# KyanChen/RSPrompter

Hardware: NVIDIA H100
Metric: images/sec (higher is better)
Workload: dtype bf16

## Files before the change

### include/rsp_b200.h

```cpp
#ifndef RSP_B200_H_
#define RSP_B200_H_

#include <stdint.h>

#ifdef __cplusplus
extern "C" {
#endif

#define RSP_ABI_VERSION 2

int rsp_abi_version(void);
const char* rsp_last_error(void);

int rsp_gemm_bf16(const void* A, int lda, const void* W, int ldw, void* out, int ldo, int M, int N,
                  int K, const float* bias, const void* residual, int ldr, int res_fp32, int res_mod,
                  const int32_t* row_map, int act, int out_fp32, void* stream);

int rsp_conv3x3_nhwc_bf16(const void* x, int B, int H, int W, int C, const void* Wt, int ldw, void* out, int ldo,
                          int N, const float* bias, const void* residual, int ldr, int res_fp32, int act,
                          int out_fp32, void* stream);
int rsp_conv3x3_geometry_ok(int B, int H, int W, int C);

int rsp_gemm_bf16_simt(const void* A, int lda, const void* W, int ldw, void* out, int ldo, int M,
                       int N, int K, const float* bias, const void* residual, int ldr, int res_fp32,
// ... 33 lines not shown
                      void* stream);

int rsp_token_self_attention(const void* q, const void* k, const void* v, void* out, int N, int T,
                             int heads, int c, void* stream);
int rsp_t2i_attention(const void* q, const void* K, const void* V, int ldkv, const int32_t* kv_block, void* out,
                      int N, int Tq, int HW, void* stream);
int rsp_i2t_attention(const void* Q, const int32_t* q_block, const void* ktok, const void* vtok,
                      void* out, int N, int Tq, int HW, void* stream);

int rsp_t2i_fused(const void* keys, int ldk, const void* kvw, const float* kvb, const void* pe_kv, const void* q,
                  void* out, int N, int Tq, int HW, void* stream);

int rsp_i2t_fused(const void* keys, int ldk, const void* wq, const float* qb, const void* pe_q, const void* ktok,
                  const void* vtok, const void* wo, const float* ob, const float* ln_g, const float* ln_b, float eps,
                  void* out, int N, int Tq, int HW, void* stream);


int rsp_rpn_decode(const float* head_out, int ld, const int64_t* topk_idx, int K, int B, int H, int W,
                   int A, int stride, const float* base_anchors, const float* stds4, float img_h, float img_w,
                   float min_size, int out_off, int out_ld, float* boxes, float* scores, void* stream);
int rsp_rpn_decode_shapes(const float* head_out, int ld, const int64_t* topk_idx, int K, int B, int H, int W, int A,
                          int stride, const float* base_anchors, const float* stds4, const float* img_shapes,
                          float min_size, int out_off, int out_ld, float* boxes, float* scores, void* stream);

int rsp_bbox_cls_decode(const float* cls, int ld_cls, const float* reg, int ld_reg, const float* rois,
                        const uint8_t* roi_valid, int n, int C, const float* stds4, float img_h, float img_w,
                        float score_thr, float* scores, float* boxes, int64_t* labels, void* stream);
int rsp_bbox_cls_decode_shapes(const float* cls, int ld_cls, const float* reg, int ld_reg, const float* rois,
                               const uint8_t* roi_valid, int n, int C, const float* stds4, const float* img_shapes,
                               float score_thr, float* scores, float* boxes, int64_t* labels, void* stream);
// ... 115 lines not shown
```

### profiles/decoder_bench.py

```python
#!/usr/bin/env python
from __future__ import annotations

import argparse
import collections
import json
import os
import subprocess
import sys

ROOT = os.path.dirname(os.path.dirname(os.path.abspath(__file__)))
if ROOT not in sys.path:
    sys.path.insert(0, ROOT)

import torch

from rsprompter_b200 import _lib, synthetic
from rsprompter_b200.sam_config import SamDecoderArch
from rsprompter_b200.sam_decoder import SamMaskDecoderB200

NQ = 100


def _card() -> dict:
    q = subprocess.run(["nvidia-smi", "--query-gpu=name,power.limit,clocks.max.sm", "--format=csv,noheader"],
# ... 57 lines not shown
    N, Tq, C = ktok.shape
    return 4.0 * N * Tq * hw * C, Q.shape[0] * C * 2 + N * hw * C * 2


def _t2i_fused_cost(q, keys, kvw, kvb, pe_kv, hw):
    N, Tq, C = q.shape
    return 2.0 * keys.shape[0] * 256 * 256 + 4.0 * N * Tq * hw * C, keys.shape[0] * 256 * 2 + 2 * _nb(q)


def _i2t_fused_cost(keys, wq, qb, pe_q, ktok, vtok, wo, ob, ln, hw):
    N, Tq, C = ktok.shape
    R = keys.shape[0]
    return 2.0 * R * 256 * 128 * 2 + 4.0 * N * Tq * hw * C, R * 256 * 2 * 2


def _family(name: str, args, kw, n_img_rows: int) -> str:
    if name == "gemm":
        a, w = args[0], args[1]
        if a.shape[0] < n_img_rows:
            return "token-side gemm"
        if kw.get("ln64_gelu") is not None:
            return "up1 gemm (LN64 + GELU)"
        if kw.get("ln") is not None:
            return "i2t out_proj gemm (+ LN4)"
        if w.shape[0] == 256:
            return "t2i k|v gemm"
        return "i2t q gemm"
    return {"gemm_upscale_mask": "up2 gemm (GELU + hyper)", "t2i_attention": "t2i attention",
            "i2t_attention": "i2t attention", "t2i_fused": "t2i fused (k|v gemm + attention)",
            "i2t_fused": "i2t fused (q gemm + attention + out_proj + LN4)"}.get(name, "token-side " + name)


COSTS = {"gemm": _gemm_cost, "gemm_upscale_mask": _upscale_cost, "t2i_attention": _t2i_cost,
         "i2t_attention": _i2t_cost, "t2i_fused": _t2i_fused_cost, "i2t_fused": _i2t_fused_cost}
WRAPPED = ("gemm", "gemm_upscale_mask", "t2i_attention", "i2t_attention", "t2i_fused", "i2t_fused", "add_cast_bf16",
           "cast_bf16", "token_self_attention")


def per_family(run, n_img_rows: int, iters: int) -> dict:
    calls = []
    orig = {k: getattr(_lib, k) for k in WRAPPED if hasattr(_lib, k)}

    def wrap(name, fn):
        def inner(*args, **kw):
            s, e = torch.cuda.Event(enable_timing=True), torch.cuda.Event(enable_timing=True)
            s.record()
            out = fn(*args, **kw)
            e.record()
            cost = COSTS[name](*args, **kw) if name in COSTS else (0.0, 0)
            calls.append((_family(name, args, kw, n_img_rows), s, e, cost))
            return out
# ... 82 lines not shown
```

### rsprompter_b200/_lib.py

```python
from __future__ import annotations

import ctypes
import os
import subprocess
from pathlib import Path

import torch

_PKG_DIR = Path(__file__).resolve().parent
LIB_PATH = _PKG_DIR / "librsp_b200.so"
CSRC_DIR = _PKG_DIR / "csrc"


class RspError(RuntimeError):
    """Raised when an ``rsp_*`` entry point returns a non-zero status."""


def build_library(verbose: bool = False) -> Path:
    cmd = ["make", "-C", str(CSRC_DIR), "-j", str(os.cpu_count() or 4), "all"]
    res = subprocess.run(cmd, capture_output=True, text=True)
    if res.returncode != 0:
        raise RuntimeError(f"building librsp_b200.so failed:\n{res.stdout[-4000:]}\n{res.stderr[-4000:]}")
    if verbose:
        print(res.stdout[-2000:])
# ... 23 lines not shown
    "rsp_layernorm": ([_vp, _i, _i, _vp, _i, _i, _vp, _vp, _vp, _i, _i, _f, _i, _vp, _i, _vp], _i),
    "rsp_patchify16": ([_vp, _vp, _i, _i, _i, _vp], _i),
    "rsp_layernorm_add": ([_vp, _vp, _i, _vp, _i, _vp, _vp, _vp, _vp, _i, _vp, ctypes.c_longlong, _i, _f, _vp], _i),
    "rsp_im2col_nhwc": ([_vp, _vp, _i, _i, _i, _i, _i, _i, _i, _i, _vp], _i),
    "rsp_nhwc_to_nchw": ([_vp, _i, _vp, _i, _i, _i, _vp], _i),
    "rsp_cast_f32_bf16": ([_vp, _vp, ctypes.c_longlong, _vp], _i),
    "rsp_add_table_bf16": ([_vp, _vp, _vp, ctypes.c_longlong, ctypes.c_longlong, _vp], _i),
    "rsp_gemm_bf16_ex": ([_vp, _i, _vp, _i, _vp, _i, _i, _i, _i, _vp, _vp, _i, _i, _i, _vp, _i, _i,
                          _i, _vp, _vp, _f, _vp, _i, _vp, _vp, _i, _i, _vp], _i),
    "rsp_add_cast_bf16": ([_vp, _vp, _vp, ctypes.c_longlong, ctypes.c_longlong, _vp], _i),
    "rsp_token_self_attention": ([_vp, _vp, _vp, _vp, _i, _i, _i, _i, _vp], _i),
    "rsp_t2i_attention": ([_vp, _vp, _vp, _i, _vp, _vp, _i, _i, _i, _vp], _i),
    "rsp_i2t_attention": ([_vp, _vp, _vp, _vp, _vp, _i, _i, _i, _vp], _i),
    "rsp_t2i_fused": ([_vp, _i, _vp, _vp, _vp, _vp, _vp, _i, _i, _i, _vp], _i),
    "rsp_i2t_fused": ([_vp, _i, _vp, _vp, _vp, _vp, _vp, _vp, _vp, _vp, _vp, _f, _vp, _i, _i, _i, _vp], _i),
    "rsp_rpn_decode": ([_vp, _i, _vp, _i, _i, _i, _i, _i, _i, _vp, _vp, _f, _f, _f, _i, _i, _vp, _vp, _vp], _i),
    "rsp_bbox_cls_decode": ([_vp, _i, _vp, _i, _vp, _vp, _i, _i, _vp, _f, _f, _f, _vp, _vp, _vp, _vp], _i),
    "rsp_rpn_decode_shapes": ([_vp, _i, _vp, _i, _i, _i, _i, _i, _i, _vp, _vp, _vp, _f, _i, _i, _vp, _vp, _vp], _i),
    "rsp_nms_batched_topk": ([_vp, _vp, _vp, _i, _i, _f, _vp, _vp, _vp, _i, _vp], _i),
    "rsp_bbox_cls_decode_shapes": ([_vp, _i, _vp, _i, _vp, _vp, _i, _i, _vp, _vp, _f, _vp, _vp, _vp, _vp], _i),
    "rsp_nms_batched": ([_vp, _vp, _vp, _i, _i, _f, _vp, _vp, _vp, _vp], _i),
    "rsp_compact_keep": ([_vp, _vp, _vp, _vp, _i, _i, _i, _vp, _vp, _vp, _vp, _vp, _vp], _i),
    "rsp_roi_align_nhwc": ([_vp, _vp, _vp, _vp, _vp, _i, _vp, _i, _i, _i, _f, _vp, _vp], _i),
    "rsp_mask_paste": ([_vp, _vp, _i, _i, _i, _i, _i, _f, _i, _vp], _i),
    "rsp_pool2_nhwc": ([_vp, _vp, _i, _i, _i, _i, _i, _vp], _i),
    "rsp_zero_border_nhwc": ([_vp, _i, _i, _i, _i, _vp], _i),
    "rsp_sigmoid_f32": ([_vp, _vp, ctypes.c_longlong, _vp], _i),
    "rsp_mask_paste_boxes": ([_vp, _vp, _vp, _i, _i, _i, _i, _i, _f, _i, _vp], _i),
    "rsp_groupnorm_nhwc": ([_vp, _vp, _vp, _vp, _vp, _vp, _i, _i, _i, _i, _i, _f, _i, _vp], _i),
    "rsp_ms_deform_attn_sample": ([_vp, _vp, _i, _vp, _vp, _i, _i, _i, _i, _vp, _vp], _i),
# ... 272 lines not shown
    assert C == 128 and hw % 64 == 0
    assert keys.dtype == torch.bfloat16 and keys.dim() == 2 and keys.stride(1) == 1 and keys.shape == (N * hw, 256)
    for t, shape in ((wq, (128, 256)), (pe_q, (hw, 128)), (ktok, (N, Tq, 128)), (vtok, (N, Tq, 128)), (wo, (256, 128))):
        assert t.dtype == torch.bfloat16 and t.shape == shape and t.is_contiguous()
    for t, n in ((qb, 128), (ob, 256), (g, 256), (b, 256)):
        assert t.dtype == torch.float32 and t.numel() == n and t.is_contiguous()
    out = torch.empty((N * hw, 256), device=keys.device, dtype=torch.bfloat16)
    _check(_lib.rsp_i2t_fused(_ptr(keys), keys.stride(0), _ptr(wq), _ptr(qb), _ptr(pe_q), _ptr(ktok), _ptr(vtok),
                              _ptr(wo), _ptr(ob), _ptr(g), _ptr(b), float(eps), _ptr(out), N, Tq, hw, _stream()),
           "rsp_i2t_fused")
    launch_count += 1
    _log("gemm", 2.0 * N * hw * 256 * 256)
    return out


def i2t_attention(Q: torch.Tensor, ktok: torch.Tensor, vtok: torch.Tensor, hw: int,
                  q_block: torch.Tensor | None = None) -> torch.Tensor:
    global launch_count
    _require_cuda(Q, ktok, vtok, q_block)
    N, Tq, C = ktok.shape
    assert C == 128 and Q.dtype == torch.bfloat16 and Q.is_contiguous() and Q.shape[1] == 128
    assert ktok.dtype == torch.bfloat16 and vtok.dtype == torch.bfloat16
    assert ktok.is_contiguous() and vtok.is_contiguous() and vtok.shape == ktok.shape
    if q_block is not None:
        assert q_block.dtype == torch.int32 and q_block.numel() == N and q_block.is_contiguous()
    else:
        assert Q.shape[0] == N * hw
    out = torch.empty((N * hw, 128), device=Q.device, dtype=torch.bfloat16)
    _check(_lib.rsp_i2t_attention(_ptr(Q), _ptr(q_block), _ptr(ktok), _ptr(vtok), _ptr(out), N, Tq, hw, _stream()),
           "rsp_i2t_attention")
# ... 811 lines not shown
```

### rsprompter_b200/csrc/abi.cu

```cuda
#include "../../include/rsp_b200.h"

#include "attention.h"
#include "gemm.h"
#include "rowops.h"

namespace rsp { const char* last_error(); }
using namespace rsp;

static inline cudaStream_t S(void* s) { return static_cast<cudaStream_t>(s); }

extern "C" {

int rsp_abi_version(void) { return RSP_ABI_VERSION; }
const char* rsp_last_error(void) { return rsp::last_error(); }

static GemmArgs make_gemm_args(const void* A, int lda, const void* W, int ldw, void* out, int ldo,
                               int M, int N, int K, const float* bias, const void* residual, int ldr,
                               int res_fp32, int res_mod, const int32_t* row_map, int act,
                               int out_fp32) {
  GemmArgs a;
  a.A = A; a.lda = lda; a.W = W; a.ldw = ldw; a.out = out; a.ldo = ldo;
  a.M = M; a.N = N; a.K = K; a.bias = bias; a.residual = residual; a.ldr = ldr;
  a.res_fp32 = res_fp32; a.res_mod = res_mod; a.row_map = row_map; a.act = act;
  a.out_fp32 = out_fp32;
// ... 146 lines not shown
                      void* out, int N, int Tq, int HW, void* stream) {
  return i2t_attention(Q, q_block, ktok, vtok, out, N, Tq, HW, S(stream));
}

int rsp_t2i_fused(const void* keys, int ldk, const void* kvw, const float* kvb, const void* pe_kv, const void* q,
                  void* out, int N, int Tq, int HW, void* stream) {
  return t2i_fused(keys, ldk, kvw, kvb, pe_kv, q, out, N, Tq, HW, S(stream));
}

int rsp_i2t_fused(const void* keys, int ldk, const void* wq, const float* qb, const void* pe_q, const void* ktok,
                  const void* vtok, const void* wo, const float* ob, const float* ln_g, const float* ln_b, float eps,
                  void* out, int N, int Tq, int HW, void* stream) {
  return i2t_fused(keys, ldk, wq, qb, pe_q, ktok, vtok, wo, ob, ln_g, ln_b, eps, out, N, Tq, HW, S(stream));
}

}

#include "detect.h"

extern "C" {

int rsp_rpn_decode(const float* head_out, int ld, const int64_t* topk_idx, int K, int B, int H, int W,
                   int A, int stride, const float* base_anchors, const float* stds4, float img_h, float img_w,
                   float min_size, int out_off, int out_ld, float* boxes, float* scores, void* stream) {
  return rpn_decode(head_out, ld, reinterpret_cast<const long long*>(topk_idx), K, B, H, W, A, stride,
                    base_anchors, stds4, img_h, img_w, nullptr, min_size, out_off, out_ld, boxes, scores, S(stream));
}

int rsp_rpn_decode_shapes(const float* head_out, int ld, const int64_t* topk_idx, int K, int B, int H, int W, int A,
                          int stride, const float* base_anchors, const float* stds4, const float* img_shapes,
// ... 222 lines not shown
```

### rsprompter_b200/csrc/decoder.cu

```cuda
#include "decoder.h"
#include "sm90.cuh"

namespace rsp {

__device__ __forceinline__ void unpack8(const uint4& u, float (&f)[8]) {
  const uint32_t w[4] = {u.x, u.y, u.z, u.w};
#pragma unroll
  for (int j = 0; j < 4; ++j) {
    const __nv_bfloat162 h = *reinterpret_cast<const __nv_bfloat162*>(&w[j]);
    f[2 * j] = __bfloat162float(h.x);
    f[2 * j + 1] = __bfloat162float(h.y);
  }
}

__global__ void add_cast_bf16_kernel(const float* __restrict__ a, const float* __restrict__ b,
                                     __nv_bfloat16* __restrict__ out, long long n, long long b_mod) {
  const long long i = (static_cast<long long>(blockIdx.x) * blockDim.x + threadIdx.x) * 4;
  if (i >= n) return;
  float4 x = *reinterpret_cast<const float4*>(a + i);
  if (b) {
    const float4 y = *reinterpret_cast<const float4*>(b + (b_mod > 0 ? i % b_mod : i));
    x.x += y.x; x.y += y.y; x.z += y.z; x.w += y.w;
  }
  *reinterpret_cast<uint2*>(out + i) = make_uint2(pack_bf16x2(x.x, x.y), pack_bf16x2(x.z, x.w));
// ... 769 lines not shown
  static bool attr_set_dev[kMaxDevices] = {};
  bool& attr_set = attr_set_dev[current_device()];
  if (!attr_set) {
    RSP_CHECK_CUDA(cudaFuncSetAttribute(i2t_fused_kernel, cudaFuncAttributeMaxDynamicSharedMemorySize, IF_SMEM));
    attr_set = true;
  }
  const int num_tiles = static_cast<int>(M / IF_TILE);
  const int grid = num_tiles < num_sms() ? num_tiles : num_sms();
  i2t_fused_kernel<<<grid, IF_THREADS, IF_SMEM, stream>>>(
      tk, to, tq, tw, qb, static_cast<const __nv_bfloat16*>(pe_q), static_cast<const __nv_bfloat16*>(ktok),
      static_cast<const __nv_bfloat16*>(vtok), ob, ln_g, ln_b, eps, Tq, HW, num_tiles, 0.25f);
  RSP_CHECK_LAUNCH();
  return RSP_OK;
}

}
```

### rsprompter_b200/csrc/decoder.h

```cpp
#pragma once
#include "host_util.h"

namespace rsp {

int add_cast_bf16(const float* a, const float* b, void* out, long long n, long long b_mod,
                  cudaStream_t stream);
int token_self_attention(const void* q, const void* k, const void* v, void* out, int N, int T,
                         int heads, int c, cudaStream_t stream);
int t2i_attention(const void* q, const void* K, const void* V, int ldkv, const int* kv_block, void* out, int N,
                  int Tq, int HW, cudaStream_t stream);
int t2i_fused(const void* keys, int ldk, const void* kvw, const float* kvb, const void* pe_kv, const void* q,
              void* out, int N, int Tq, int HW, cudaStream_t stream);
int i2t_attention(const void* Q, const int* q_block, const void* ktok, const void* vtok, void* out,
                  int N, int Tq, int HW, cudaStream_t stream);
int i2t_fused(const void* keys, int ldk, const void* wq, const float* qb, const void* pe_q, const void* ktok,
              const void* vtok, const void* wo, const float* ob, const float* ln_g, const float* ln_b, float eps,
              void* out, int N, int Tq, int HW, cudaStream_t stream);

}
```

### rsprompter_b200/csrc/gemm_v2.cu

```cuda
#include <cstdlib>

#include "gemm.h"
#include "sm90.cuh"

namespace rsp {

namespace v2 {

constexpr int BM = 128;
constexpr int BK = 64;
constexpr int A_BYTES = BM * BK * 2;
constexpr int STG_ROW = 136;
constexpr int STG_WARP = 32 * STG_ROW;
constexpr int BAR_BYTES = 256;
constexpr int SMEM_MAX = 227 * 1024;

enum { EPI_STD = 0, EPI_LN_ROW = 1, EPI_LN64_GELU = 2, EPI_GELU_HYPER = 3 };

template <int BN, int EPI>
struct Cfg {
  static constexpr bool SPLIT = EPI == EPI_STD;
  static_assert(!SPLIT || BN <= 128, "a 64 x 256 wgmma needs more registers than a 512-thread block has per thread");
  static constexpr int THREADS = SPLIT ? 512 : 384;
  static constexpr int EPI_WARPS = SPLIT ? 4 : 8;
// ... 80 lines not shown
    float hyp[32];
    {
      const float4* h4 = reinterpret_cast<const float4*>(p.hyper + static_cast<size_t>(n) * 32);
#pragma unroll
      for (int i = 0; i < 8; ++i) {
        const float4 h = __ldg(h4 + i);
        hyp[4 * i] = h.x; hyp[4 * i + 1] = h.y; hyp[4 * i + 2] = h.z; hyp[4 * i + 3] = h.w;
      }
    }
    const uint32_t t_row = acc_row(acc_base, C::ACC_LD, q * 32 + lane) + 4 * hf * 64;
    float m2[2];
#pragma unroll
    for (int t = 0; t < 2; ++t) {
      uint32_t r[32];
      acc_ld32(t_row + (t * 32) * 4, r);
      const float4* b4 = reinterpret_cast<const float4*>(p.bias + hf * 64 + t * 32);
      float acc = 0.f;
#pragma unroll
      for (int i = 0; i < 8; ++i) {
        const float4 b = __ldg(b4 + i);
        acc += gelu_fast(__uint_as_float(r[4 * i]) + b.x) * hyp[4 * i];
        acc += gelu_fast(__uint_as_float(r[4 * i + 1]) + b.y) * hyp[4 * i + 1];
        acc += gelu_fast(__uint_as_float(r[4 * i + 2]) + b.z) * hyp[4 * i + 2];
        acc += gelu_fast(__uint_as_float(r[4 * i + 3]) + b.w) * hyp[4 * i + 3];
      }
      m2[t] = acc;
    }
    if (valid) {
      const int W4 = 4 * p.grid_w;
      const int Y = 4 * y + 2 * (tap1 >> 1) + hf, X = 4 * x + 2 * (tap1 & 1);
      *reinterpret_cast<float2*>(p.mask_out + (static_cast<size_t>(n) * 4 * p.grid_h + Y) * W4 + X) =
          make_float2(m2[0], m2[1]);
    }
  } else if constexpr (EPI == EPI_LN_ROW) {
    const uint32_t t_row = acc_row(acc_base, C::ACC_LD, q * 32 + lane) + 4 * hf * 128;
    const int col_warp = hf * 128;
    const int row0 = m_blk * BM + q * 32;
    const uint32_t sbuf = smem_u32(stg_all) + e * 4096;
    const uint32_t srow = sbuf + lane * 128;
    const int sw = lane & 7;
    float2* xchg = reinterpret_cast<float2*>(stg_all + 8 * 4096);
// ... 105 lines not shown
    const uint32_t t_row = acc_row(acc_base, C::ACC_LD, q * 32 + lane) + 4 * hf * C::COLS_PER_WARP;
    const int col_warp = n_blk * BN + hf * C::COLS_PER_WARP;
    const int sub = lane >> 4, cl = lane & 15;
#pragma unroll 1
    for (int gi = 0; gi < C::COLS_PER_WARP / 64; ++gi) {
      const int col0 = col_warp + gi * 64;
      if (col0 >= p.N) break;
      float v[64];
      {
        uint32_t r0[32], r1[32];
        acc_ld32(t_row + (gi * 64) * 4, r0);
        acc_ld32(t_row + (gi * 64 + 32) * 4, r1);
#pragma unroll
        for (int i = 0; i < 32; ++i) { v[i] = __uint_as_float(r0[i]); v[32 + i] = __uint_as_float(r1[i]); }
      }
      float sum = 0.f;
#pragma unroll
      for (int i = 0; i < 16; ++i) {
        const float4 b = __ldg(reinterpret_cast<const float4*>(p.bias + col0) + i);
        v[4 * i] += b.x; v[4 * i + 1] += b.y; v[4 * i + 2] += b.z; v[4 * i + 3] += b.w;
        sum += v[4 * i] + v[4 * i + 1] + v[4 * i + 2] + v[4 * i + 3];
      }
      const float mean = sum * (1.0f / 64.0f);
      float var = 0.f;
#pragma unroll
      for (int i = 0; i < 64; ++i) { const float d = v[i] - mean; var += d * d; }
      const float rstd = rsqrtf(var * (1.0f / 64.0f) + p.ln_eps);
      if (p.tma_store) {
        const uint32_t sbuf = smem_u32(stg_all) + e * 4096;
        const uint32_t srow = sbuf + lane * 128;
        const int sw = lane & 7;
        uint32_t pk[32];
#pragma unroll
        for (int i = 0; i < 16; ++i) {
          const float4 g = __ldg(reinterpret_cast<const float4*>(p.ln_gamma) + i);
          const float4 bt = __ldg(reinterpret_cast<const float4*>(p.ln_beta) + i);
          const float y0 = gelu_fast((v[4 * i] - mean) * rstd * g.x + bt.x);
          const float y1 = gelu_fast((v[4 * i + 1] - mean) * rstd * g.y + bt.y);
          const float y2 = gelu_fast((v[4 * i + 2] - mean) * rstd * g.z + bt.z);
          const float y3 = gelu_fast((v[4 * i + 3] - mean) * rstd * g.w + bt.w);
          pk[2 * i] = pack_bf16x2(y0, y1);
          pk[2 * i + 1] = pack_bf16x2(y2, y3);
        }
        if (lane == 0) bulk_wait_read0();
        __syncwarp();
#pragma unroll
        for (int j = 0; j < 8; ++j)
          asm volatile("st.shared.v4.b32 [%0], {%1, %2, %3, %4};" ::"r"(srow + ((j ^ sw) << 4)), "r"(pk[4 * j]),
                       "r"(pk[4 * j + 1]), "r"(pk[4 * j + 2]), "r"(pk[4 * j + 3])
                       : "memory");
        fence_proxy_async_smem();
        __syncwarp();
        if (lane == 0) { tma_store_2d(&tma_c, sbuf, col0, m_blk * BM + q * 32); bulk_commit(); }
        continue;
      }
      const uint32_t a = stg_s + lane * STG_ROW;
#pragma unroll
      for (int i = 0; i < 16; ++i) {
        const float4 g = __ldg(reinterpret_cast<const float4*>(p.ln_gamma) + i);
        const float4 bt = __ldg(reinterpret_cast<const float4*>(p.ln_beta) + i);
        const float y0 = gelu_fast((v[4 * i] - mean) * rstd * g.x + bt.x);
        const float y1 = gelu_fast((v[4 * i + 1] - mean) * rstd * g.y + bt.y);
        const float y2 = gelu_fast((v[4 * i + 2] - mean) * rstd * g.z + bt.z);
        const float y3 = gelu_fast((v[4 * i + 3] - mean) * rstd * g.w + bt.w);
        asm volatile("st.shared.v2.b32 [%0], {%1, %2};" ::"r"(a + i * 8), "r"(pack_bf16x2(y0, y1)),
                     "r"(pack_bf16x2(y2, y3))
                     : "memory");
      }
      __syncwarp();
      const int col = col0 + cl * 4;
#pragma unroll 4
      for (int k = 0; k < 16; ++k) {
        const int rr = 2 * k + sub;
        const int orow = __shfl_sync(0xffffffffu, my_orow, rr);
        if (orow < 0) continue;
        uint32_t w0, w1;
        asm volatile("ld.shared.v2.b32 {%0, %1}, [%2];" : "=r"(w0), "=r"(w1) : "r"(stg_s + rr * STG_ROW + cl * 8));
        *reinterpret_cast<uint2*>(static_cast<__nv_bfloat16*>(p.out) + static_cast<size_t>(orow) * p.ldo + col) =
            make_uint2(w0, w1);
// ... 539 lines not shown
```

### rsprompter_b200/csrc/sm90.cuh

```cuda
#pragma once
#include <cuda.h>
#include <cuda_bf16.h>
#include <cuda_runtime.h>
#include <stdint.h>

namespace rsp {

__device__ __forceinline__ uint32_t smem_u32(const void* p) {
  return static_cast<uint32_t>(__cvta_generic_to_shared(p));
}

__device__ __forceinline__ uint32_t elect_one() {
  uint32_t pred = 0;
  asm volatile(
      "{\n"
      ".reg .b32 rx;\n"
      ".reg .pred px;\n"
      "elect.sync rx|px, 0xffffffff;\n"
      "selp.u32 %0, 1, 0, px;\n"
      "}\n"
      : "=r"(pred));
  return pred;
}

// ... 249 lines not shown
        "+f"(d[32]), "+f"(d[33]), "+f"(d[34]), "+f"(d[35]), "+f"(d[36]), "+f"(d[37]), "+f"(d[38]), "+f"(d[39]),
        "+f"(d[40]), "+f"(d[41]), "+f"(d[42]), "+f"(d[43]), "+f"(d[44]), "+f"(d[45]), "+f"(d[46]), "+f"(d[47]),
        "+f"(d[48]), "+f"(d[49]), "+f"(d[50]), "+f"(d[51]), "+f"(d[52]), "+f"(d[53]), "+f"(d[54]), "+f"(d[55]),
        "+f"(d[56]), "+f"(d[57]), "+f"(d[58]), "+f"(d[59]), "+f"(d[60]), "+f"(d[61]), "+f"(d[62]), "+f"(d[63]),
        "+f"(d[64]), "+f"(d[65]), "+f"(d[66]), "+f"(d[67]), "+f"(d[68]), "+f"(d[69]), "+f"(d[70]), "+f"(d[71]),
        "+f"(d[72]), "+f"(d[73]), "+f"(d[74]), "+f"(d[75]), "+f"(d[76]), "+f"(d[77]), "+f"(d[78]), "+f"(d[79]),
        "+f"(d[80]), "+f"(d[81]), "+f"(d[82]), "+f"(d[83]), "+f"(d[84]), "+f"(d[85]), "+f"(d[86]), "+f"(d[87]),
        "+f"(d[88]), "+f"(d[89]), "+f"(d[90]), "+f"(d[91]), "+f"(d[92]), "+f"(d[93]), "+f"(d[94]), "+f"(d[95]),
        "+f"(d[96]), "+f"(d[97]), "+f"(d[98]), "+f"(d[99]), "+f"(d[100]), "+f"(d[101]), "+f"(d[102]), "+f"(d[103]),
        "+f"(d[104]), "+f"(d[105]), "+f"(d[106]), "+f"(d[107]), "+f"(d[108]), "+f"(d[109]), "+f"(d[110]), "+f"(d[111]),
        "+f"(d[112]), "+f"(d[113]), "+f"(d[114]), "+f"(d[115]), "+f"(d[116]), "+f"(d[117]), "+f"(d[118]), "+f"(d[119]),
        "+f"(d[120]), "+f"(d[121]), "+f"(d[122]), "+f"(d[123]), "+f"(d[124]), "+f"(d[125]), "+f"(d[126]), "+f"(d[127])
      : "r"(a[0]), "r"(a[1]), "r"(a[2]), "r"(a[3]), "l"(b), "r"(acc));
}

__device__ __forceinline__ uint32_t acc_row(uint32_t base, int ld, int row) {
  return base + static_cast<uint32_t>(row * ld) * 4u;
}
__device__ __forceinline__ void acc_ld32(uint32_t addr, uint32_t (&r)[32]) {
#pragma unroll
  for (int i = 0; i < 8; ++i)
    asm volatile("ld.shared.v4.b32 {%0, %1, %2, %3}, [%4];"
                 : "=r"(r[4 * i]), "=r"(r[4 * i + 1]), "=r"(r[4 * i + 2]), "=r"(r[4 * i + 3])
                 : "r"(addr + 16 * i));
}
__device__ __forceinline__ void acc_st32(uint32_t addr, const uint32_t (&r)[32]) {
#pragma unroll
  for (int i = 0; i < 8; ++i)
    asm volatile("st.shared.v4.b32 [%0], {%1, %2, %3, %4};" ::"r"(addr + 16 * i), "r"(r[4 * i]), "r"(r[4 * i + 1]),
                 "r"(r[4 * i + 2]), "r"(r[4 * i + 3])
// ... 71 lines not shown
__device__ __forceinline__ float gelu_erf(float x) {
  return 0.5f * x * (1.0f + erff(x * 0.70710678118654752440f));
}

__device__ __forceinline__ float gelu_fast(float x) {
  const float x2 = x * x;
  float p = fmaf(3.229002131292087e-06f, x2, -8.823835998556129e-05f);
  p = fmaf(p, x2, -0.0003602734064506858f);
  p = fmaf(p, x2, 0.10522668605353103f);
  p = fmaf(p, x2, 2.302045390974673f);
  float e;
  asm("ex2.approx.ftz.f32 %0, %1;" : "=f"(e) : "f"(-p * x));
  return __fdividef(x, 1.0f + e);
}

}
```

### rsprompter_b200/sam_decoder.py

```python
from __future__ import annotations

import math

import torch
from torch import nn

from . import _lib
from .registry import MODELS, BaseModule
from .sam_config import SamDecoderArch, decoder_arch, vision_arch
from .sam_encoder import _Affine, _load_pretrained


class _Embedding(nn.Module):
    def __init__(self, n: int, c: int):
        super().__init__()
        self.weight = nn.Parameter(torch.empty(n, c), requires_grad=False)


class _SamAttention(nn.Module):
    def __init__(self, C: int, internal: int):
        super().__init__()
        self.q_proj = _Affine((internal, C))
        self.k_proj = _Affine((internal, C))
        self.v_proj = _Affine((internal, C))
# ... 210 lines not shown
            ktok = _lib.gemm(qin, i2t["kw"], i2t["kb"])
            vtok = _lib.gemm(_lib.cast_bf16(queries), i2t["vw"], i2t["vb"])
            if kblk is None and HW % 64 == 0:
                keys_b = _lib.i2t_fused(keys_b, i2t["qw"], i2t["qb"], pt["q"][li], ktok.view(N, Tt, -1),
                                        vtok.view(N, Tt, -1), i2t["ow"], i2t["ob"], (*L["ln4"], a.layer_norm_eps), HW)
            else:
                Qimg = _lib.gemm(keys_b, i2t["qw"], i2t["qb"], residual=pt["q"][li], res_mod=HW)
                att = _lib.i2t_attention(Qimg, ktok.view(N, Tt, -1), vtok.view(N, Tt, -1), HW, q_block=kblk)
                keys_b = _lib.gemm(att, i2t["ow"], i2t["ob"], residual=keys_res, ln=(*L["ln4"], a.layer_norm_eps),
                                   res_block_map=kblk, res_block_rows=HW if kblk is not None else 0)
            keys_res, kblk = keys_b, None
        queries = t2i(p["final"], queries, keys_b, pt["kv"][-1], None, (*p["lnf"], 1e-5))
        qv = queries.view(N, Tt, C)
        iou_tok = _lib.cast_bf16(qv[:, 0].contiguous())
        iou = self._ff(iou_tok, p["iou"])
        up1 = _lib.gemm(keys_b, p["up1_w"], p["up1_b"], ln64_gelu=(*p["up_ln"], 1e-6))
        up1 = up1.view(N * HW * 4, -1)
        sel = range(1, self.num_mask_tokens) if multimask_output else range(0, 1)
        masks = []
        for i in sel:
            mt = _lib.cast_bf16(qv[:, 1 + i].contiguous())
            hyper = self._ff(mt, p["hyper"][i])
            masks.append(_lib.gemm_upscale_mask(up1, p["up2_w"], p["up2_b"], hyper, h, w))
        masks = torch.stack(masks, dim=1) if len(masks) > 1 else masks[0].unsqueeze(1)
        iou = iou[:, 1:] if multimask_output else iou[:, 0:1]
        return masks, iou

    def forward(self, image_embeddings, image_positional_embeddings, sparse_prompt_embeddings,
                dense_prompt_embeddings, multimask_output, attention_similarity=None,
                target_embedding=None, output_attentions=None):
        if attention_similarity is not None or target_embedding is not None:
            raise NotImplementedError("attention_similarity / target_embedding are not used by RSPrompter")
        N, C, h, w = image_embeddings.shape
        assert sparse_prompt_embeddings.shape[1] == 1, "point_batch_size must be 1"
        to_rows = lambda t: t.to(torch.float32).permute(0, 2, 3, 1).reshape(-1, C).contiguous()
        pos_rows = to_rows(image_positional_embeddings[:1])
        masks, iou = self.decode(to_rows(image_embeddings), pos_rows, sparse_prompt_embeddings[:, 0],
                                 (h, w), dense_rows=to_rows(dense_prompt_embeddings),
                                 multimask_output=multimask_output)
# ... 97 lines not shown
```

Baseline: 61.05.

## Fuse mask upscaler up1 GEMM, LN64+GELU, up2 GEMM and hyper dot into one kernel

After: 61.61 (median of 6 runs). Within noise of the previous version (+0.9%).

```diff
diff --git a/include/rsp_b200.h b/include/rsp_b200.h
--- a/include/rsp_b200.h
+++ b/include/rsp_b200.h
@@ -71,6 +71,10 @@
 int rsp_i2t_fused(const void* keys, int ldk, const void* wq, const float* qb, const void* pe_q, const void* ktok,
                   const void* vtok, const void* wo, const float* ob, const float* ln_g, const float* ln_b, float eps,
                   void* out, int N, int Tq, int HW, void* stream);
+
+int rsp_upscale_mask_fused(const void* keys, int ldk, const void* w1, const float* b1, const float* ln_g,
+                           const float* ln_b, float eps, const void* w2, const float* b2, const float* hyper, float* masks,
+                           int N, int n_out, int h, int w, void* stream);
 
 
 int rsp_rpn_decode(const float* head_out, int ld, const int64_t* topk_idx, int K, int B, int H, int W,
diff --git a/profiles/decoder_bench.py b/profiles/decoder_bench.py
--- a/profiles/decoder_bench.py
+++ b/profiles/decoder_bench.py
@@ -95,6 +95,12 @@
     return 2.0 * R * 256 * 128 * 2 + 4.0 * N * Tq * hw * C, R * 256 * 2 * 2
 
 
+def _upscale_fused_cost(keys, w1, b1, ln, w2, b2, hyper, gh, gw):
+    R = keys.shape[0]
+    N, n_out, _ = hyper.shape
+    return 2.0 * R * 256 * 256 + 2.0 * R * 4 * 64 * 128, R * 256 * 2 + N * n_out * 16 * gh * gw * 4
+
+
 def _family(name: str, args, kw, n_img_rows: int) -> str:
     if name == "gemm":
         a, w = args[0], args[1]
@@ -109,13 +115,15 @@
         return "i2t q gemm"
     return {"gemm_upscale_mask": "up2 gemm (GELU + hyper)", "t2i_attention": "t2i attention",
             "i2t_attention": "i2t attention", "t2i_fused": "t2i fused (k|v gemm + attention)",
-            "i2t_fused": "i2t fused (q gemm + attention + out_proj + LN4)"}.get(name, "token-side " + name)
+            "i2t_fused": "i2t fused (q gemm + attention + out_proj + LN4)",
+            "upscale_mask_fused": "upscaler fused (up1 + LN64 + GELU + up2 + GELU + hyper)"}.get(name, "token-side " + name)
 
 
 COSTS = {"gemm": _gemm_cost, "gemm_upscale_mask": _upscale_cost, "t2i_attention": _t2i_cost,
-         "i2t_attention": _i2t_cost, "t2i_fused": _t2i_fused_cost, "i2t_fused": _i2t_fused_cost}
-WRAPPED = ("gemm", "gemm_upscale_mask", "t2i_attention", "i2t_attention", "t2i_fused", "i2t_fused", "add_cast_bf16",
-           "cast_bf16", "token_self_attention")
+         "i2t_attention": _i2t_cost, "t2i_fused": _t2i_fused_cost, "i2t_fused": _i2t_fused_cost,
+         "upscale_mask_fused": _upscale_fused_cost}
+WRAPPED = ("gemm", "gemm_upscale_mask", "t2i_attention", "i2t_attention", "t2i_fused", "i2t_fused", "upscale_mask_fused",
+           "add_cast_bf16", "cast_bf16", "token_self_attention")
 
 
 def per_family(run, n_img_rows: int, iters: int) -> dict:
diff --git a/rsprompter_b200/_lib.py b/rsprompter_b200/_lib.py
--- a/rsprompter_b200/_lib.py
+++ b/rsprompter_b200/_lib.py
@@ -61,6 +61,7 @@
     "rsp_i2t_attention": ([_vp, _vp, _vp, _vp, _vp, _i, _i, _i, _vp], _i),
     "rsp_t2i_fused": ([_vp, _i, _vp, _vp, _vp, _vp, _vp, _i, _i, _i, _vp], _i),
     "rsp_i2t_fused": ([_vp, _i, _vp, _vp, _vp, _vp, _vp, _vp, _vp, _vp, _vp, _f, _vp, _i, _i, _i, _vp], _i),
+    "rsp_upscale_mask_fused": ([_vp, _i, _vp, _vp, _vp, _vp, _f, _vp, _vp, _vp, _vp, _i, _i, _i, _i, _vp], _i),
     "rsp_rpn_decode": ([_vp, _i, _vp, _i, _i, _i, _i, _i, _i, _vp, _vp, _f, _f, _f, _i, _i, _vp, _vp, _vp], _i),
     "rsp_bbox_cls_decode": ([_vp, _i, _vp, _i, _vp, _vp, _i, _i, _vp, _f, _f, _f, _vp, _vp, _vp, _vp], _i),
     "rsp_rpn_decode_shapes": ([_vp, _i, _vp, _i, _i, _i, _i, _i, _i, _vp, _vp, _vp, _f, _i, _i, _vp, _vp, _vp], _i),
@@ -363,6 +364,28 @@
     return out
 
 
+def upscale_mask_fused(keys: torch.Tensor, w1: torch.Tensor, b1: torch.Tensor, ln: tuple, w2: torch.Tensor,
+                       b2: torch.Tensor, hyper: torch.Tensor, grid_h: int, grid_w: int) -> torch.Tensor:
+    global launch_count
+    g, b, eps = ln
+    _require_cuda(keys, w1, b1, g, b, w2, b2, hyper)
+    N, n_out, C = hyper.shape
+    hw = grid_h * grid_w
+    assert C == 32 and hw % 64 == 0 and hyper.dtype == torch.float32 and hyper.is_contiguous()
+    assert keys.dtype == torch.bfloat16 and keys.dim() == 2 and keys.stride(1) == 1 and keys.shape == (N * hw, 256)
+    for t, shape in ((w1, (256, 256)), (w2, (128, 64))):
+        assert t.dtype == torch.bfloat16 and t.shape == shape and t.is_contiguous()
+    for t, n in ((b1, 256), (g, 64), (b, 64), (b2, 128)):
+        assert t.dtype == torch.float32 and t.numel() == n and t.is_contiguous()
+    out = torch.empty((N, n_out, 4 * grid_h, 4 * grid_w), device=keys.device, dtype=torch.float32)
+    _check(_lib.rsp_upscale_mask_fused(_ptr(keys), keys.stride(0), _ptr(w1), _ptr(b1), _ptr(g), _ptr(b), float(eps),
+                                       _ptr(w2), _ptr(b2), _ptr(hyper), _ptr(out), N, n_out, grid_h, grid_w, _stream()),
+           "rsp_upscale_mask_fused")
+    launch_count += 1
+    _log("gemm", 2.0 * N * hw * 256 * 256 + 2.0 * N * hw * 4 * 64 * 128)
+    return out
+
+
 def i2t_attention(Q: torch.Tensor, ktok: torch.Tensor, vtok: torch.Tensor, hw: int,
                   q_block: torch.Tensor | None = None) -> torch.Tensor:
     global launch_count
diff --git a/rsprompter_b200/csrc/abi.cu b/rsprompter_b200/csrc/abi.cu
--- a/rsprompter_b200/csrc/abi.cu
+++ b/rsprompter_b200/csrc/abi.cu
@@ -184,6 +184,12 @@
   return i2t_fused(keys, ldk, wq, qb, pe_q, ktok, vtok, wo, ob, ln_g, ln_b, eps, out, N, Tq, HW, S(stream));
 }
 
+int rsp_upscale_mask_fused(const void* keys, int ldk, const void* w1, const float* b1, const float* ln_g,
+                           const float* ln_b, float eps, const void* w2, const float* b2, const float* hyper, float* masks,
+                           int N, int n_out, int h, int w, void* stream) {
+  return upscale_mask_fused(keys, ldk, w1, b1, ln_g, ln_b, eps, w2, b2, hyper, masks, N, n_out, h, w, S(stream));
+}
+
 }
 
 #include "detect.h"
diff --git a/rsprompter_b200/csrc/decoder.cu b/rsprompter_b200/csrc/decoder.cu
--- a/rsprompter_b200/csrc/decoder.cu
+++ b/rsprompter_b200/csrc/decoder.cu
@@ -807,4 +807,238 @@
   return RSP_OK;
 }
 
-}
+constexpr int UF_THREADS = 256;
+constexpr int UF_TILE = 64;
+constexpr int UF_MAX_OUT = 4;
+constexpr int UF_W1_BYTES = 4 * 256 * 128;
+constexpr int UF_W2_BYTES = 128 * 128;
+constexpr int UF_A_BYTES = 4 * UF_TILE * 128;
+constexpr int UF_A_OFF = UF_W1_BYTES + UF_W2_BYTES;
+constexpr int UF_VEC_OFF = UF_A_OFF + 2 * UF_A_BYTES;
+constexpr int UF_BAR_OFF = UF_VEC_OFF + 512 * 4;
+constexpr int UF_SMEM = UF_BAR_OFF + 64;
+static_assert(UF_SMEM <= 227 * 1024, "upscale_mask_fused shared memory");
+
+__global__ void __launch_bounds__(UF_THREADS, 1)
+upscale_mask_fused_kernel(const __grid_constant__ CUtensorMap tma_keys,
+                          const __grid_constant__ CUtensorMap tma_w1,
+                          const __nv_bfloat16* __restrict__ w2,
+                          const float* __restrict__ b1,
+                          const float* __restrict__ ln_g, const float* __restrict__ ln_b, float eps,
+                          const float* __restrict__ b2,
+                          const float* __restrict__ hyper,
+                          float* __restrict__ masks,
+                          int n_out, int gh, int gw, int num_tiles) {
+  extern __shared__ __align__(1024) uint8_t smem[];
+  const uint32_t s_w1 = smem_u32(smem);
+  const uint32_t s_w2 = s_w1 + UF_W1_BYTES;
+  const uint32_t s_a = s_w1 + UF_A_OFF;
+  float* vec = reinterpret_cast<float*>(smem + UF_VEC_OFF);
+  const float* s_b1 = vec;
+  const float* s_g = vec + 256;
+  const float* s_bt = vec + 320;
+  const float* s_b2 = vec + 384;
+  uint64_t* bars = reinterpret_cast<uint64_t*>(smem + UF_BAR_OFF);
+  const uint32_t bar_w = smem_u32(&bars[0]);
+  const int warp = threadIdx.x >> 5, lane = threadIdx.x & 31;
+  const int wg = warp >> 2;
+  const int tw = threadIdx.x & 127;
+  const uint32_t bar_full = smem_u32(&bars[1 + wg]);
+  const uint32_t sa = s_a + wg * UF_A_BYTES;
+  const int stride = 2 * gridDim.x;
+  const int HW = gh * gw;
+  auto load_tile = [&](int tile) {
+    mbar_expect_tx(bar_full, UF_A_BYTES);
+    for (int kb = 0; kb < 4; ++kb) tma_load_2d(sa + kb * (UF_TILE * 128), &tma_keys, bar_full, kb * 64, tile * UF_TILE);
+  };
+
+  for (int i = threadIdx.x; i < 256; i += UF_THREADS) {
+    vec[i] = b1[i];
+    if (i < 64) { vec[256 + i] = ln_g[i]; vec[320 + i] = ln_b[i]; }
+    if (i < 128) vec[384 + i] = b2[i];
+  }
+  for (int i = threadIdx.x; i < 128 * 8; i += UF_THREADS) {
+    const int n = i >> 3, c = i & 7;
+    const int src = 32 * ((n & 7) >> 1) + 2 * (n >> 3) + (n & 1);
+    const uint4 v = *reinterpret_cast<const uint4*>(w2 + src * 64 + c * 8);
+    asm volatile("st.shared.v4.b32 [%0], {%1, %2, %3, %4};" ::"r"(s_w2 + n * 128 + ((c ^ (n & 7)) << 4)), "r"(v.x),
+                 "r"(v.y), "r"(v.z), "r"(v.w)
+                 : "memory");
+  }
+  fence_proxy_async_smem();
+  if (threadIdx.x == 0) {
+    tma_prefetch_desc(&tma_keys);
+    for (int b = 0; b < 3; ++b) mbar_init(smem_u32(&bars[b]), 1);
+    fence_barrier_init();
+  }
+  __syncthreads();
+  if (threadIdx.x == 0) {
+    mbar_expect_tx(bar_w, UF_W1_BYTES);
+    for (int kb = 0; kb < 4; ++kb) tma_load_2d(s_w1 + kb * (256 * 128), &tma_w1, bar_w, kb * 64, 0);
+  }
+  const int first = blockIdx.x + wg * gridDim.x;
+  if (tw == 0 && first < num_tiles) load_tile(first);
+  const int g = lane >> 2, t = lane & 3;
+  const int frow = (warp & 3) * 16 + g;
+  const bool odd = t & 1;
+  mbar_wait(bar_w, 0);
+  uint32_t phase = 0;
+#pragma unroll 1
+  for (int tile = first; tile < num_tiles; tile += stride, phase ^= 1) {
+    const int row0 = tile * UF_TILE;
+    const int p = row0 / HW;
+    const int prow = row0 - p * HW + frow + (odd ? 8 : 0);
+    const int py = prow / gw, px = prow - py * gw;
+    mbar_wait(bar_full, phase);
+#pragma unroll 1
+    for (int h = 0; h < 2; ++h) {
+      uint32_t af[2][4][4];
+      {
+        float acc[64];
+        wgmma_fence();
+#pragma unroll
+        for (int kb = 0; kb < 4; ++kb) {
+#pragma unroll
+          for (int k = 0; k < 4; ++k)
+            Wgmma<128>::ss<0>(acc, make_gdesc(sa + kb * (UF_TILE * 128) + k * 32, 16, 1024),
+                              make_gdesc(s_w1 + kb * (256 * 128) + h * (128 * 128) + k * 32, 16, 1024), (kb | k) != 0);
+        }
+        wgmma_commit();
+        wgmma_wait<0>();
+        acc_fence(acc);
+        if (h == 1) {
+          named_bar_sync(1 + wg, 128);
+          if (tw == 0 && tile + stride < num_tiles) load_tile(tile + stride);
+        }
+#pragma unroll
+        for (int j = 0; j < 16; ++j) {
+          const float2 b = *reinterpret_cast<const float2*>(s_b1 + h * 128 + 8 * j + 2 * t);
+          acc[4 * j] += b.x; acc[4 * j + 1] += b.y; acc[4 * j + 2] += b.x; acc[4 * j + 3] += b.y;
+        }
+        float vg[64];
+#pragma unroll
+        for (int jj = 0; jj < 8; ++jj) {
+          float rc[4][2];
+#pragma unroll
+          for (int r = 0; r < 4; ++r) {
+            const int cs = (t - r) & 3;
+            const int src = (lane & ~3) | ((t + r) & 3);
+#pragma unroll
+            for (int e = 0; e < 2; ++e) {
+              const float mine = sel4(cs, acc[4 * jj + e], acc[4 * jj + 2 + e], acc[4 * (8 + jj) + e],
+                                      acc[4 * (8 + jj) + 2 + e]);
+              rc[r][e] = __shfl_sync(0xffffffffu, mine, src);
+            }
+          }
+#pragma unroll
+          for (int s = 0; s < 4; ++s) {
+            const int r = (s - t) & 3;
+#pragma unroll
+            for (int e = 0; e < 2; ++e) vg[8 * jj + 2 * s + e] = sel4(r, rc[0][e], rc[1][e], rc[2][e], rc[3][e]);
+          }
+        }
+        float mean, rstd;
+        ln64_stats(vg, eps, mean, rstd);
+        float mu[4], rs[4];
+#pragma unroll
+        for (int c = 0; c < 4; ++c) {
+          mu[c] = __shfl_sync(0xffffffffu, mean, (lane & ~3) | c);
+          rs[c] = __shfl_sync(0xffffffffu, rstd, (lane & ~3) | c);
+        }
+#pragma unroll
+        for (int tau = 0; tau < 2; ++tau) {
+#pragma unroll
+          for (int jj = 0; jj < 8; ++jj) {
+            const int j = 8 * tau + jj;
+            const float2 gm = *reinterpret_cast<const float2*>(s_g + 8 * jj + 2 * t);
+            const float2 bt = *reinterpret_cast<const float2*>(s_bt + 8 * jj + 2 * t);
+            const int c0 = 2 * tau, c1 = 2 * tau + 1;
+            const uint32_t lo = pack_bf16x2(ln64_gelu(acc[4 * j], mu[c0], rs[c0], gm.x, bt.x),
+                                            ln64_gelu(acc[4 * j + 1], mu[c0], rs[c0], gm.y, bt.y));
+            const uint32_t hi = pack_bf16x2(ln64_gelu(acc[4 * j + 2], mu[c1], rs[c1], gm.x, bt.x),
+                                            ln64_gelu(acc[4 * j + 3], mu[c1], rs[c1], gm.y, bt.y));
+            af[tau][jj >> 1][(jj & 1) * 2] = lo;
+            af[tau][jj >> 1][(jj & 1) * 2 + 1] = hi;
+          }
+        }
+      }
+      float m[UF_MAX_OUT][2][2];
+#pragma unroll
+      for (int tau = 0; tau < 2; ++tau) {
+        float acc[64];
+        wgmma_fence();
+#pragma unroll
+        for (int c = 0; c < 4; ++c) wgmma_rs_bf16_n128(acc, af[tau][c], make_gdesc(s_w2 + c * 32, 16, 1024), c != 0);
+        wgmma_commit();
+        wgmma_wait<0>();
+        acc_fence(acc);
+#pragma unroll
+        for (int rr = 0; rr < 2; ++rr) {
+          float x[32];
+#pragma unroll
+          for (int j = 0; j < 16; ++j) { x[2 * j] = acc[4 * j + 2 * rr]; x[2 * j + 1] = acc[4 * j + 2 * rr + 1]; }
+          gelu_bias32(x, s_b2 + 32 * t);
+#pragma unroll
+          for (int o = 0; o < UF_MAX_OUT; ++o) {
+            if (o < n_out) {
+              float hyp[32];
+              const float4* h4 = reinterpret_cast<const float4*>(hyper + (static_cast<size_t>(p) * n_out + o) * 32);
+#pragma unroll
+              for (int i = 0; i < 8; ++i) {
+                const float4 hv = __ldg(h4 + i);
+                hyp[4 * i] = hv.x; hyp[4 * i + 1] = hv.y; hyp[4 * i + 2] = hv.z; hyp[4 * i + 3] = hv.w;
+              }
+              m[o][tau][rr] = hyper_dot32(x, hyp);
+            }
+          }
+        }
+      }
+      const int Y = 4 * py + 2 * h + (t >> 1);
+#pragma unroll
+      for (int o = 0; o < UF_MAX_OUT; ++o) {
+        if (o < n_out) {
+          const float r0 = __shfl_xor_sync(0xffffffffu, odd ? m[o][0][0] : m[o][0][1], 1);
+          const float r1 = __shfl_xor_sync(0xffffffffu, odd ? m[o][1][0] : m[o][1][1], 1);
+          const float4 val = odd ? make_float4(r0, m[o][0][1], r1, m[o][1][1]) : make_float4(m[o][0][0], r0, m[o][1][0], r1);
+          *reinterpret_cast<float4*>(masks + ((static_cast<size_t>(p) * n_out + o) * 4 * gh + Y) * (4 * gw) + 4 * px) =
+              val;
+        }
+      }
+    }
+  }
+}
+
+int upscale_mask_fused(const void* keys, int ldk, const void* w1, const float* b1, const float* ln_g, const float* ln_b,
+                       float eps, const void* w2, const float* b2, const float* hyper, float* masks, int N, int n_out,
+                       int h, int w, cudaStream_t stream) {
+  RSP_CHECK_ARG(keys && w1 && b1 && ln_g && ln_b && w2 && b2 && hyper && masks, "upscale_mask_fused: null pointer");
+  RSP_CHECK_ARG(N > 0 && n_out > 0 && n_out <= UF_MAX_OUT && h > 0 && w > 0 &&
+                static_cast<long long>(h) * w % UF_TILE == 0 && static_cast<long long>(N) * h * w < (1ll << 31),
+                "upscale_mask_fused: N %d, n_out %d, grid %d x %d (n_out <= 4, h * w %% 64 == 0, N * h * w < 2^31)", N,
+                n_out, h, w);
+  RSP_CHECK_ARG(ldk >= 256 && ldk % 8 == 0, "upscale_mask_fused: keys row stride %d", ldk);
+  const uintptr_t a16 = reinterpret_cast<uintptr_t>(keys) | reinterpret_cast<uintptr_t>(w1) |
+                        reinterpret_cast<uintptr_t>(w2) | reinterpret_cast<uintptr_t>(hyper) |
+                        reinterpret_cast<uintptr_t>(masks);
+  const uintptr_t a4 = reinterpret_cast<uintptr_t>(b1) | reinterpret_cast<uintptr_t>(ln_g) |
+                       reinterpret_cast<uintptr_t>(ln_b) | reinterpret_cast<uintptr_t>(b2);
+  RSP_CHECK_ARG((a16 & 15) == 0 && (a4 & 3) == 0, "upscale_mask_fused: operand alignment");
+  const uint64_t M = static_cast<uint64_t>(N) * h * w;
+  CUtensorMap tk, tw1;
+  RSP_TRY(make_tmap_bf16_2d(&tk, keys, M, 256, static_cast<uint64_t>(ldk) * 2, UF_TILE, 64));
+  RSP_TRY(make_tmap_bf16_2d(&tw1, w1, 256, 256, 256 * 2, 256, 64));
+  static bool attr_set_dev[kMaxDevices] = {};
+  bool& attr_set = attr_set_dev[current_device()];
+  if (!attr_set) {
+    RSP_CHECK_CUDA(cudaFuncSetAttribute(upscale_mask_fused_kernel, cudaFuncAttributeMaxDynamicSharedMemorySize, UF_SMEM));
+    attr_set = true;
+  }
+  const int num_tiles = static_cast<int>(M / UF_TILE);
+  const int grid = num_tiles < num_sms() ? num_tiles : num_sms();
+  upscale_mask_fused_kernel<<<grid, UF_THREADS, UF_SMEM, stream>>>(
+      tk, tw1, static_cast<const __nv_bfloat16*>(w2), b1, ln_g, ln_b, eps, b2, hyper, masks, n_out, h, w, num_tiles);
+  RSP_CHECK_LAUNCH();
+  return RSP_OK;
+}
+
+}
diff --git a/rsprompter_b200/csrc/decoder.h b/rsprompter_b200/csrc/decoder.h
--- a/rsprompter_b200/csrc/decoder.h
+++ b/rsprompter_b200/csrc/decoder.h
@@ -16,5 +16,8 @@
 int i2t_fused(const void* keys, int ldk, const void* wq, const float* qb, const void* pe_q, const void* ktok,
               const void* vtok, const void* wo, const float* ob, const float* ln_g, const float* ln_b, float eps,
               void* out, int N, int Tq, int HW, cudaStream_t stream);
+int upscale_mask_fused(const void* keys, int ldk, const void* w1, const float* b1, const float* ln_g, const float* ln_b,
+                       float eps, const void* w2, const float* b2, const float* hyper, float* masks, int N, int n_out,
+                       int h, int w, cudaStream_t stream);
 
 }
diff --git a/rsprompter_b200/csrc/gemm_v2.cu b/rsprompter_b200/csrc/gemm_v2.cu
--- a/rsprompter_b200/csrc/gemm_v2.cu
+++ b/rsprompter_b200/csrc/gemm_v2.cu
@@ -118,17 +118,11 @@
     for (int t = 0; t < 2; ++t) {
       uint32_t r[32];
       acc_ld32(t_row + (t * 32) * 4, r);
-      const float4* b4 = reinterpret_cast<const float4*>(p.bias + hf * 64 + t * 32);
-      float acc = 0.f;
-#pragma unroll
-      for (int i = 0; i < 8; ++i) {
-        const float4 b = __ldg(b4 + i);
-        acc += gelu_fast(__uint_as_float(r[4 * i]) + b.x) * hyp[4 * i];
-        acc += gelu_fast(__uint_as_float(r[4 * i + 1]) + b.y) * hyp[4 * i + 1];
-        acc += gelu_fast(__uint_as_float(r[4 * i + 2]) + b.z) * hyp[4 * i + 2];
-        acc += gelu_fast(__uint_as_float(r[4 * i + 3]) + b.w) * hyp[4 * i + 3];
-      }
-      m2[t] = acc;
+      float x[32];
+#pragma unroll
+      for (int i = 0; i < 32; ++i) x[i] = __uint_as_float(r[i]);
+      gelu_bias32(x, p.bias + hf * 64 + t * 32);
+      m2[t] = hyper_dot32(x, hyp);
     }
     if (valid) {
       const int W4 = 4 * p.grid_w;
@@ -264,18 +258,13 @@
 #pragma unroll
         for (int i = 0; i < 32; ++i) { v[i] = __uint_as_float(r0[i]); v[32 + i] = __uint_as_float(r1[i]); }
       }
-      float sum = 0.f;
 #pragma unroll
       for (int i = 0; i < 16; ++i) {
         const float4 b = __ldg(reinterpret_cast<const float4*>(p.bias + col0) + i);
         v[4 * i] += b.x; v[4 * i + 1] += b.y; v[4 * i + 2] += b.z; v[4 * i + 3] += b.w;
-        sum += v[4 * i] + v[4 * i + 1] + v[4 * i + 2] + v[4 * i + 3];
-      }
-      const float mean = sum * (1.0f / 64.0f);
-      float var = 0.f;
-#pragma unroll
-      for (int i = 0; i < 64; ++i) { const float d = v[i] - mean; var += d * d; }
-      const float rstd = rsqrtf(var * (1.0f / 64.0f) + p.ln_eps);
+      }
+      float mean, rstd;
+      ln64_stats(v, p.ln_eps, mean, rstd);
       if (p.tma_store) {
         const uint32_t sbuf = smem_u32(stg_all) + e * 4096;
         const uint32_t srow = sbuf + lane * 128;
@@ -285,10 +274,10 @@
         for (int i = 0; i < 16; ++i) {
           const float4 g = __ldg(reinterpret_cast<const float4*>(p.ln_gamma) + i);
           const float4 bt = __ldg(reinterpret_cast<const float4*>(p.ln_beta) + i);
-          const float y0 = gelu_fast((v[4 * i] - mean) * rstd * g.x + bt.x);
-          const float y1 = gelu_fast((v[4 * i + 1] - mean) * rstd * g.y + bt.y);
-          const float y2 = gelu_fast((v[4 * i + 2] - mean) * rstd * g.z + bt.z);
-          const float y3 = gelu_fast((v[4 * i + 3] - mean) * rstd * g.w + bt.w);
+          const float y0 = ln64_gelu(v[4 * i], mean, rstd, g.x, bt.x);
+          const float y1 = ln64_gelu(v[4 * i + 1], mean, rstd, g.y, bt.y);
+          const float y2 = ln64_gelu(v[4 * i + 2], mean, rstd, g.z, bt.z);
+          const float y3 = ln64_gelu(v[4 * i + 3], mean, rstd, g.w, bt.w);
           pk[2 * i] = pack_bf16x2(y0, y1);
           pk[2 * i + 1] = pack_bf16x2(y2, y3);
         }
@@ -309,10 +298,10 @@
       for (int i = 0; i < 16; ++i) {
         const float4 g = __ldg(reinterpret_cast<const float4*>(p.ln_gamma) + i);
         const float4 bt = __ldg(reinterpret_cast<const float4*>(p.ln_beta) + i);
-        const float y0 = gelu_fast((v[4 * i] - mean) * rstd * g.x + bt.x);
-        const float y1 = gelu_fast((v[4 * i + 1] - mean) * rstd * g.y + bt.y);
-        const float y2 = gelu_fast((v[4 * i + 2] - mean) * rstd * g.z + bt.z);
-        const float y3 = gelu_fast((v[4 * i + 3] - mean) * rstd * g.w + bt.w);
+        const float y0 = ln64_gelu(v[4 * i], mean, rstd, g.x, bt.x);
+        const float y1 = ln64_gelu(v[4 * i + 1], mean, rstd, g.y, bt.y);
+        const float y2 = ln64_gelu(v[4 * i + 2], mean, rstd, g.z, bt.z);
+        const float y3 = ln64_gelu(v[4 * i + 3], mean, rstd, g.w, bt.w);
         asm volatile("st.shared.v2.b32 [%0], {%1, %2};" ::"r"(a + i * 8), "r"(pack_bf16x2(y0, y1)),
                      "r"(pack_bf16x2(y2, y3))
                      : "memory");
diff --git a/rsprompter_b200/csrc/sm90.cuh b/rsprompter_b200/csrc/sm90.cuh
--- a/rsprompter_b200/csrc/sm90.cuh
+++ b/rsprompter_b200/csrc/sm90.cuh
@@ -287,6 +287,28 @@
       : "r"(a[0]), "r"(a[1]), "r"(a[2]), "r"(a[3]), "l"(b), "r"(acc));
 }
 
+__device__ __forceinline__ void wgmma_rs_bf16_n128(float (&d)[64], const uint32_t (&a)[4], uint64_t b, uint32_t acc) {
+  asm volatile(
+      "{\n.reg .pred p;\n"
+      "setp.ne.b32 p, %69, 0;\n"
+      "wgmma.mma_async.sync.aligned.m64n128k16.f32.bf16.bf16 "
+      "{"
+      "%0, %1, %2, %3, %4, %5, %6, %7, %8, %9, %10, %11, %12, %13, %14, %15, "
+      "%16, %17, %18, %19, %20, %21, %22, %23, %24, %25, %26, %27, %28, %29, %30, %31, "
+      "%32, %33, %34, %35, %36, %37, %38, %39, %40, %41, %42, %43, %44, %45, %46, %47, "
+      "%48, %49, %50, %51, %52, %53, %54, %55, %56, %57, %58, %59, %60, %61, %62, %63"
+      "}, {%64, %65, %66, %67}, %68, p, 1, 1, 0;\n}\n"
+      : "+f"(d[0]), "+f"(d[1]), "+f"(d[2]), "+f"(d[3]), "+f"(d[4]), "+f"(d[5]), "+f"(d[6]), "+f"(d[7]),
+        "+f"(d[8]), "+f"(d[9]), "+f"(d[10]), "+f"(d[11]), "+f"(d[12]), "+f"(d[13]), "+f"(d[14]), "+f"(d[15]),
+        "+f"(d[16]), "+f"(d[17]), "+f"(d[18]), "+f"(d[19]), "+f"(d[20]), "+f"(d[21]), "+f"(d[22]), "+f"(d[23]),
+        "+f"(d[24]), "+f"(d[25]), "+f"(d[26]), "+f"(d[27]), "+f"(d[28]), "+f"(d[29]), "+f"(d[30]), "+f"(d[31]),
+        "+f"(d[32]), "+f"(d[33]), "+f"(d[34]), "+f"(d[35]), "+f"(d[36]), "+f"(d[37]), "+f"(d[38]), "+f"(d[39]),
+        "+f"(d[40]), "+f"(d[41]), "+f"(d[42]), "+f"(d[43]), "+f"(d[44]), "+f"(d[45]), "+f"(d[46]), "+f"(d[47]),
+        "+f"(d[48]), "+f"(d[49]), "+f"(d[50]), "+f"(d[51]), "+f"(d[52]), "+f"(d[53]), "+f"(d[54]), "+f"(d[55]),
+        "+f"(d[56]), "+f"(d[57]), "+f"(d[58]), "+f"(d[59]), "+f"(d[60]), "+f"(d[61]), "+f"(d[62]), "+f"(d[63])
+      : "r"(a[0]), "r"(a[1]), "r"(a[2]), "r"(a[3]), "l"(b), "r"(acc));
+}
+
 __device__ __forceinline__ uint32_t acc_row(uint32_t base, int ld, int row) {
   return base + static_cast<uint32_t>(row * ld) * 4u;
 }
@@ -388,4 +410,34 @@
   return __fdividef(x, 1.0f + e);
 }
 
-}
+__device__ __forceinline__ void ln64_stats(const float (&v)[64], float eps, float& mean, float& rstd) {
+  float sum = 0.f;
+#pragma unroll
+  for (int i = 0; i < 16; ++i) sum += v[4 * i] + v[4 * i + 1] + v[4 * i + 2] + v[4 * i + 3];
+  mean = sum * (1.0f / 64.0f);
+  float var = 0.f;
+#pragma unroll
+  for (int i = 0; i < 64; ++i) { const float d = v[i] - mean; var += d * d; }
+  rstd = rsqrtf(var * (1.0f / 64.0f) + eps);
+}
+__device__ __forceinline__ float ln64_gelu(float v, float mean, float rstd, float g, float b) {
+  return gelu_fast((v - mean) * rstd * g + b);
+}
+__device__ __forceinline__ void gelu_bias32(float (&x)[32], const float* b) {
+#pragma unroll
+  for (int i = 0; i < 8; ++i) {
+    const float4 bb = reinterpret_cast<const float4*>(b)[i];
+    x[4 * i] = gelu_fast(x[4 * i] + bb.x);
+    x[4 * i + 1] = gelu_fast(x[4 * i + 1] + bb.y);
+    x[4 * i + 2] = gelu_fast(x[4 * i + 2] + bb.z);
+    x[4 * i + 3] = gelu_fast(x[4 * i + 3] + bb.w);
+  }
+}
+__device__ __forceinline__ float hyper_dot32(const float (&x)[32], const float (&hyp)[32]) {
+  float acc = 0.f;
+#pragma unroll
+  for (int i = 0; i < 32; ++i) acc += x[i] * hyp[i];
+  return acc;
+}
+
+}
diff --git a/rsprompter_b200/sam_decoder.py b/rsprompter_b200/sam_decoder.py
--- a/rsprompter_b200/sam_decoder.py
+++ b/rsprompter_b200/sam_decoder.py
@@ -248,15 +248,16 @@
         qv = queries.view(N, Tt, C)
         iou_tok = _lib.cast_bf16(qv[:, 0].contiguous())
         iou = self._ff(iou_tok, p["iou"])
-        up1 = _lib.gemm(keys_b, p["up1_w"], p["up1_b"], ln64_gelu=(*p["up_ln"], 1e-6))
-        up1 = up1.view(N * HW * 4, -1)
         sel = range(1, self.num_mask_tokens) if multimask_output else range(0, 1)
-        masks = []
-        for i in sel:
-            mt = _lib.cast_bf16(qv[:, 1 + i].contiguous())
-            hyper = self._ff(mt, p["hyper"][i])
-            masks.append(_lib.gemm_upscale_mask(up1, p["up2_w"], p["up2_b"], hyper, h, w))
-        masks = torch.stack(masks, dim=1) if len(masks) > 1 else masks[0].unsqueeze(1)
+        hypers = [self._ff(_lib.cast_bf16(qv[:, 1 + i].contiguous()), p["hyper"][i]) for i in sel]
+        if kblk is None and HW % 64 == 0 and w % 2 == 0:
+            masks = _lib.upscale_mask_fused(keys_b, p["up1_w"], p["up1_b"], (*p["up_ln"], 1e-6), p["up2_w"],
+                                            p["up2_b"], torch.stack(hypers, dim=1), h, w)
+        else:
+            up1 = _lib.gemm(keys_b, p["up1_w"], p["up1_b"], ln64_gelu=(*p["up_ln"], 1e-6))
+            up1 = up1.view(N * HW * 4, -1)
+            masks = [_lib.gemm_upscale_mask(up1, p["up2_w"], p["up2_b"], hyper, h, w) for hyper in hypers]
+            masks = torch.stack(masks, dim=1) if len(masks) > 1 else masks[0].unsqueeze(1)
         iou = iou[:, 1:] if multimask_output else iou[:, 0:1]
         return masks, iou
 
```
